# ModelCloud/GPTQModel

Hardware: NVIDIA H100
Metric: W4A16 g128 QuantLinear: decode tok/s + prefill TFLOPS vs HBM/TC roofline (higher is better)
Workload: dtype f16

## Files before the change

gptqmodel_b200/csrc/b2q_gemm.cu:

```cuda
#include <cuda.h>

#include "b2q_common.cuh"
#include "b2q_dequant.cuh"
#include "b2q_gemm.cuh"
#include "b2q_internal.h"
#include "b2q_wgmma.cuh"

namespace b2q {

template <typename T, int BITS, bool ASYM, int STAGES>
__global__ void __launch_bounds__(G_THREADS, 1)
    gemm_kernel(const __grid_constant__ CUtensorMap tmap_x, const __grid_constant__ GemmSets S, int M, int K,
                int gshc) {
  using C = GemmCfg<BITS, STAGES>;
  using E = ET<T>;
  extern __shared__ uint8_t smem_raw[];
  const uint32_t smem_base = (smem_u32(smem_raw) + 1023u) & ~1023u;
  uint8_t* smem = smem_raw + (smem_base - smem_u32(smem_raw));

  const uint32_t sA = smem_base;
  const uint32_t sB = sA + STAGES * C::A_BYTES;
  const uint32_t sP = sB + STAGES * C::B_BYTES;
  const uint32_t sBar = sP + STAGES * C::P_BYTES;
  const uint32_t bar_full = sBar, bar_bready = sBar + 8 * STAGES, bar_empty = sBar + 16 * STAGES;

  int set = 0, tn = blockIdx.x;
  if (S.nsets > 1 && tn >= S.tn_end[0]) {
    set = (S.nsets > 2 && tn >= S.tn_end[1]) ? 2 : 1;
    tn -= S.tn_end[set - 1];
  }
  const int N = S.N[set];
  const uint4* __restrict__ packed = S.packed[set];
  const T* __restrict__ scales = reinterpret_cast<const T*>(S.scales[set]);
  const uint32_t* __restrict__ qzeros = S.qzeros[set];

  const int warp = threadIdx.x >> 5, lane = threadIdx.x & 31;
  const int NT = N >> 5;
  const int n0 = tn * G_BN, m0 = blockIdx.y * G_BM;
  const int nt0 = n0 >> 5;
  const int ntiles = min(4, NT - nt0);
  const int nkb = K / G_BK;

  if (threadIdx.x == 0) {
    prefetch_tmap(&tmap_x);
    for (int s = 0; s < STAGES; ++s) {
      mbar_init(bar_full + 8 * s, 1);
      mbar_init(bar_bready + 8 * s, G_DQ_THREADS);
      mbar_init(bar_empty + 8 * s, 1);
    }
    fence_mbar_init();
  }
  __syncthreads();

  if (warp == 8) {
    if (lane == 0) {
      const int FT = N >> 4, ft0 = n0 >> 4;
      const uint32_t pbytes4 = (uint32_t)min(8, FT - ft0) * 512u;
      const uint32_t pbytes8 = (uint32_t)ntiles * C::SUB * 512u;
      for (int kb = 0; kb < nkb; ++kb) {
        const int s = kb % STAGES;
        const uint32_t ph = (kb / STAGES) & 1;
        mbar_wait(bar_empty + 8 * s, ph ^ 1);
        const int g0 = (2 * kb) >> gshc, g1 = (2 * kb + 1) >> gshc;
        const int nrows = (g1 != g0) ? 2 : 1;
        const uint32_t sbytes = (uint32_t)min(G_BN, N - n0) * 2u, zbytes = ASYM ? sbytes / 4u : 0u;
        mbar_expect_tx(bar_full + 8 * s,
                       C::A_BYTES + (BITS == 4 ? pbytes4 + nrows * (sbytes + zbytes) : 2 * pbytes8));
        tma_load_2d(sA + s * C::A_BYTES, &tmap_x, bar_full + 8 * s, kb * G_BK, m0);
        if (BITS == 4) {
          bulk_load(sP + s * C::P_BYTES, packed + ((size_t)kb * FT + ft0) * 32, pbytes4, bar_full + 8 * s);
          for (int r = 0; r < nrows; ++r) {
            const int gr = r ? g1 : g0;
            bulk_load(sP + s * C::P_BYTES + 4096 + r * 320, scales + (size_t)gr * N + n0, sbytes, bar_full + 8 * s);
            if (ASYM)
              bulk_load(sP + s * C::P_BYTES + 4096 + r * 320 + 256, qzeros + (size_t)gr * (N >> 3) + (n0 >> 3),
                        zbytes, bar_full + 8 * s);
          }
        } else {
#pragma unroll
          for (int j = 0; j < 2; ++j)
            bulk_load(sP + s * C::P_BYTES + j * C::P_CHUNK_BYTES,
                      packed + ((size_t)(kb * 2 + j) * NT + nt0) * C::SUB * 32, pbytes8, bar_full + 8 * s);
        }
      }
    }
  } else if (warp < 4) {
    float acc[2][G_BN / 2];
#pragma unroll
    for (int mb = 0; mb < 2; ++mb)
#pragma unroll
      for (int i = 0; i < G_BN / 2; ++i) acc[mb][i] = 0.f;
    for (int kb = 0; kb < nkb; ++kb) {
      const int s = kb % STAGES;
      const uint32_t ph = (kb / STAGES) & 1;
      mbar_wait(bar_full + 8 * s, ph);
      mbar_wait(bar_bready + 8 * s, ph);
      wgmma_fence();
      const uint64_t bdesc = wgmma_desc_k_sw128(sB + s * C::B_BYTES);
      const uint64_t adesc = wgmma_desc_k_sw128(sA + s * C::A_BYTES);
#pragma unroll
      for (int k = 0; k < G_BK / 16; ++k) {
#pragma unroll
        for (int mb = 0; mb < 2; ++mb)
          Wgmma<E::FMT, G_BN>::mma(acc[mb], adesc + 512 * mb + 2 * k, bdesc + 2 * k, (kb | k) != 0 ? 1u : 0u);
      }
      wgmma_commit();
      wgmma_wait<1>();
      if (kb > 0 && threadIdx.x == 0) mbar_arrive(bar_empty + 8 * ((kb - 1) % STAGES));
    }
    wgmma_wait<0>();
#pragma unroll
    for (int mb = 0; mb < 2; ++mb) wgmma_fence_regs(acc[mb]);

    const T* __restrict__ bias = reinterpret_cast<const T*>(S.bias[set]);
    T* __restrict__ out = reinterpret_cast<T*>(S.out[set]);
#pragma unroll
    for (int mb = 0; mb < 2; ++mb) {
#pragma unroll
      for (int h = 0; h < 2; ++h) {
        const int row = m0 + 64 * mb + 16 * warp + (lane >> 2) + 8 * h;
        if (row >= M) continue;
        T* dst = out + (size_t)row * N;
#pragma unroll
        for (int j = 0; j < G_BN / 8; ++j) {
          const int col = n0 + 8 * j + 2 * (lane & 3);
          if (col >= N) continue;
          float f0 = acc[mb][4 * j + 2 * h], f1 = acc[mb][4 * j + 2 * h + 1];
          if (bias != nullptr) {
            f0 = E::to_f(E::from_f(f0)) + E::to_f(bias[col]);
            f1 = E::to_f(E::from_f(f1)) + E::to_f(bias[col + 1]);
          }
          *reinterpret_cast<uint32_t*>(dst + col) = E::pack2(f0, f1);
        }
      }
    }
  } else {
    const int t = threadIdx.x - G_MMA_THREADS;
    constexpr int PF = 32 / BITS;
    constexpr int ZSYM = 1 << (BITS - 1);
    if (BITS == 4) {
      const int lp = t & 31, g = lp >> 2, tt = lp & 3;
      int f[4];
      f[0] = (t >> 5) * 16 + g;
      f[1] = f[0] + 8;
      f[2] = f[0] + 64;
      f[3] = f[0] + 72;
      for (int kb = 0; kb < nkb; ++kb) {
        const int s = kb % STAGES;
        const uint32_t ph = (kb / STAGES) & 1;
        mbar_wait(bar_full + 8 * s, ph);
        const uint8_t* pst = smem + (sP - smem_base) + s * C::P_BYTES;
        const uint4* pj = reinterpret_cast<const uint4*>(pst);
        const int grow = ((2 * kb + (tt >> 1)) >> gshc) - ((2 * kb) >> gshc);
        const uint8_t* srow = pst + 4096 + grow * 320;
#pragma unroll
        for (int u = 0; u < 2; ++u) {
          const uint4 pv = pj[t + u * 128];
          const uint32_t s_lo = *reinterpret_cast<const uint16_t*>(srow + f[2 * u] * 2);
          const uint32_t s_hi = *reinterpret_cast<const uint16_t*>(srow + f[2 * u + 1] * 2);
          int zl = ZSYM, zh = ZSYM;
          if (ASYM) {
            const uint32_t zwl = *reinterpret_cast<const uint32_t*>(srow + 256 + (f[2 * u] >> 3) * 4);
            const uint32_t zwh = *reinterpret_cast<const uint32_t*>(srow + 256 + (f[2 * u + 1] >> 3) * 4);
            zl = (int)((zwl >> (4 * g)) & 15u);
            zh = (int)((zwh >> (4 * g)) & 15u);
          }
          uint4 lo[2], hi[2];
          Dequant<T, 4>::run(pv, s_lo, zl, s_hi, zh, lo, hi);
          const uint32_t sw = (uint32_t)g;
          const uint32_t rlo = sB + s * C::B_BYTES + f[2 * u] * 128;
          const uint32_t rhi = rlo + 8 * 128;
#pragma unroll
          for (int c = 0; c < 2; ++c) {
            const uint32_t off = (((uint32_t)(2 * tt + c)) ^ sw) << 4;
            asm volatile("st.shared.v4.u32 [%0], {%1,%2,%3,%4};" ::"r"(rlo + off), "r"(lo[c].x), "r"(lo[c].y),
                         "r"(lo[c].z), "r"(lo[c].w)
                         : "memory");
            asm volatile("st.shared.v4.u32 [%0], {%1,%2,%3,%4};" ::"r"(rhi + off), "r"(hi[c].x), "r"(hi[c].y),
                         "r"(hi[c].z), "r"(hi[c].w)
                         : "memory");
          }
        }
        fence_proxy_async_smem();
        mbar_arrive(bar_bready + 8 * s);
      }
    } else {
      const int n = n0 + t;
      const int nsafe = (n < N) ? n : 0;
      const int ntl = t >> 5;
      SZRaw cur[2], nxt[2];
      cur[0] = load_sz<T, BITS, ASYM>(scales, qzeros, 0, nsafe, N);
      cur[1] = load_sz<T, BITS, ASYM>(scales, qzeros, 1 >> gshc, nsafe, N);
      for (int kb = 0; kb < nkb; ++kb) {
        const int s = kb % STAGES;
        const uint32_t ph = (kb / STAGES) & 1;
        if (kb + 1 < nkb) {
          nxt[0] = load_sz<T, BITS, ASYM>(scales, qzeros, (2 * kb + 2) >> gshc, nsafe, N);
          nxt[1] = load_sz<T, BITS, ASYM>(scales, qzeros, (2 * kb + 3) >> gshc, nsafe, N);
        }
        mbar_wait(bar_full + 8 * s, ph);
        const uint32_t brow = sB + s * C::B_BYTES + t * 128;
        const uint32_t sw = (uint32_t)(t & 7);
#pragma unroll
        for (int j = 0; j < 2; ++j) {
          int z = ZSYM;
          if (ASYM) z = (int)((cur[j].zw >> (BITS * (nsafe % PF))) & ((1u << BITS) - 1));
          const uint4* pj = reinterpret_cast<const uint4*>(smem + (sP - smem_base) + s * C::P_BYTES +
                                                           j * C::P_CHUNK_BYTES);
#pragma unroll
          for (int h = 0; h < 2; ++h) {
            const uint4 pv = pj[(ntl * 2 + h) * 32 + lane];
            uint4 o[2];
            Dequant<T, 8>::run(pv, cur[j].s, z, o);
#pragma unroll
            for (int c = 0; c < 2; ++c) {
              const uint32_t addr = brow + (((uint32_t)(j * 4 + h * 2 + c) ^ sw) << 4);
              asm volatile("st.shared.v4.u32 [%0], {%1,%2,%3,%4};" ::"r"(addr), "r"(o[c].x), "r"(o[c].y),
                           "r"(o[c].z), "r"(o[c].w)
                           : "memory");
            }
          }
        }
        fence_proxy_async_smem();
        mbar_arrive(bar_bready + 8 * s);
        cur[0] = nxt[0];
        cur[1] = nxt[1];
      }
    }
  }
}

typedef CUresult (*EncodeTiledFn)(CUtensorMap*, CUtensorMapDataType, cuuint32_t, void*, const cuuint64_t*,
                                  const cuuint64_t*, const cuuint32_t*, const cuuint32_t*, CUtensorMapInterleave,
                                  CUtensorMapSwizzle, CUtensorMapL2promotion, CUtensorMapFloatOOBfill);

static EncodeTiledFn get_encode_fn() {
  static EncodeTiledFn fn = nullptr;
  if (fn == nullptr) {
    void* p = nullptr;
    cudaDriverEntryPointQueryResult qres;
    if (cudaGetDriverEntryPoint("cuTensorMapEncodeTiled", &p, cudaEnableDefault, &qres) == cudaSuccess &&
        qres == cudaDriverEntryPointSuccess)
      fn = reinterpret_cast<EncodeTiledFn>(p);
  }
  return fn;
}

int make_x_tmap_box(CUtensorMap* map, const void* x, int M, int K, int dtype, int box_rows) {
  struct Entry {
    const void* x;
    int M, K, dtype, box;
    CUtensorMap map;
  };
  constexpr int NCACHE = 16;
  static thread_local Entry cache[NCACHE];
  static thread_local int next = 0, filled = 0;
  for (int i = 0; i < filled; ++i) {
    const Entry& c = cache[i];
    if (c.x == x && c.M == M && c.K == K && c.dtype == dtype && c.box == box_rows) {
      *map = c.map;
      return 0;
    }
  }
  EncodeTiledFn enc = get_encode_fn();
  if (enc == nullptr) {
    set_error("b2q_gemm: cuTensorMapEncodeTiled not available from the driver");
    return -1;
  }
  cuuint64_t gdim[2] = {(cuuint64_t)K, (cuuint64_t)M};
  cuuint64_t gstride[1] = {(cuuint64_t)K * 2};
  cuuint32_t box[2] = {(cuuint32_t)G_BK, (cuuint32_t)box_rows};
  cuuint32_t estr[2] = {1, 1};
  CUresult r = enc(map, dtype == 0 ? CU_TENSOR_MAP_DATA_TYPE_FLOAT16 : CU_TENSOR_MAP_DATA_TYPE_BFLOAT16, 2,
                   const_cast<void*>(x), gdim, gstride, box, estr, CU_TENSOR_MAP_INTERLEAVE_NONE,
                   CU_TENSOR_MAP_SWIZZLE_128B, CU_TENSOR_MAP_L2_PROMOTION_L2_256B,
                   CU_TENSOR_MAP_FLOAT_OOB_FILL_NONE);
  if (r != CUDA_SUCCESS) {
    set_error("b2q_gemm: cuTensorMapEncodeTiled failed (%d) for x=%p M=%d K=%d box=%d", (int)r, x, M, K, box_rows);
    return -1;
  }
  Entry& e = cache[next];
  e.x = x;
  e.M = M;
  e.K = K;
  e.dtype = dtype;
  e.box = box_rows;
  e.map = *map;
  next = (next + 1) % NCACHE;
  if (filled < NCACHE) ++filled;
  return 0;
}

int make_x_tmap(CUtensorMap* map, const void* x, int M, int K, int dtype) {
  return make_x_tmap_box(map, x, M, K, dtype, 128);
}

int gemm_gshc(const MmArgs& a) {
  if (a.group_size == 32) return 0;
  if (a.group_size == 64) return 1;
  if (a.group_size == 128) return 2;
  return 31;
}


template <typename T, int BITS, bool ASYM, int STAGES>
static int launch_gemm_t(const MmArgs& a, const void* x, const GemmSets& S) {
  using C = GemmCfg<BITS, STAGES>;
  CUtensorMap tmap;
  if (make_x_tmap(&tmap, x, a.M, a.K, a.dtype) != 0) return -1;
  auto kern = gemm_kernel<T, BITS, ASYM, STAGES>;
  static uint32_t smem_ok = 0;
  if (int e = ensure_dyn_smem(kern, C::SMEM_BYTES, smem_ok, "b2q_gemm")) return e;
  dim3 grid(S.tn_end[S.nsets - 1], (a.M + G_BM - 1) / G_BM, 1);
  kern<<<grid, G_THREADS, C::SMEM_BYTES, a.stream>>>(tmap, S, a.M, a.K, gemm_gshc(a));
  return (int)cudaGetLastError();
}

static int launch_gemm_sets(const MmArgs& a, const void* x, const GemmSets& S) {
  const bool asym = S.qzeros[0] != nullptr;
#define B2Q_GEMM_CASE(T, BITS, ST) \
  (asym ? launch_gemm_t<T, BITS, true, ST>(a, x, S) : launch_gemm_t<T, BITS, false, ST>(a, x, S))
  if (a.dtype == 0) return a.bits == 4 ? B2Q_GEMM_CASE(__half, 4, 4) : B2Q_GEMM_CASE(__half, 8, 4);
  return a.bits == 4 ? B2Q_GEMM_CASE(__nv_bfloat16, 4, 4) : B2Q_GEMM_CASE(__nv_bfloat16, 8, 4);
#undef B2Q_GEMM_CASE
}

int launch_gemm_multi(const MmArgs& a, const void* x, int nsets, const void* const* packed, const void* const* scales,
                      const int32_t* const* qzeros, const void* const* bias, void* const* out, const int* Ns) {
  if (nsets < 1 || nsets > G_MAX_SETS) {
    set_error("b2q_gemm_multi: nsets=%d out of range (1..%d)", nsets, G_MAX_SETS);
    return -1;
  }
  if (a.K % G_BK != 0) {
    set_error("b2q_gemm_multi: K=%d must be a multiple of %d", a.K, G_BK);
    return -1;
  }
  GemmSets S = {};
  S.nsets = nsets;
  int tn = 0;
  for (int i = 0; i < nsets; ++i) {
    if (Ns[i] <= 0 || Ns[i] % 32 != 0 || packed[i] == nullptr || scales[i] == nullptr || out[i] == nullptr ||
        ((qzeros[i] != nullptr) != (qzeros[0] != nullptr))) {
      set_error("b2q_gemm_multi: set %d unsupported (N=%d; all sets share K, group size and symmetry)", i, Ns[i]);
      return -1;
    }
    tn += (Ns[i] + G_BN - 1) / G_BN;
    S.tn_end[i] = tn;
    S.N[i] = Ns[i];
    S.packed[i] = (const uint4*)packed[i];
    S.scales[i] = scales[i];
    S.qzeros[i] = (const uint32_t*)qzeros[i];
    S.bias[i] = bias[i];
    S.out[i] = out[i];
  }
  for (int i = nsets; i < G_MAX_SETS; ++i) S.tn_end[i] = tn;
  return launch_gemm_sets(a, x, S);
}

int launch_gemm(const MmArgs& a) {
  if (a.K % G_BK != 0) {
    set_error("b2q_gemm: K=%d must be a multiple of %d", a.K, G_BK);
    return -1;
  }
  const void* x = a.x;
  if (a.perm != nullptr) {
    const size_t need = (size_t)a.M * a.K * 2;
    if (a.workspace == nullptr || a.workspace_bytes < need) {
      set_error("b2q_gemm: act-order needs a %zu-byte workspace (got %zu)", need, a.workspace_bytes);
      return -1;
    }
    int e = launch_permute_cols(a.x, a.perm, a.workspace, a.M, a.K, a.stream);
    if (e != 0) return e;
    x = a.workspace;
  }
  if (a.M <= 128 && env().midm && midm_supported(a)) return launch_midm(a, x);
  const void* packed = a.packed;
  const void* scales = a.scales;
  const int32_t* qzeros = (const int32_t*)a.qzeros;
  const void* bias = a.bias;
  void* out = a.out;
  return launch_gemm_multi(a, x, 1, &packed, &scales, &qzeros, &bias, &out, &a.N);
}

}
```

gptqmodel_b200/csrc/b2q_gemm.cuh:

```cuda
#pragma once
#include "b2q_common.cuh"

namespace b2q {

constexpr int G_BM = 128;
constexpr int G_BN = 128;
constexpr int G_BK = 64;
constexpr int G_MMA_THREADS = 128;
constexpr int G_DQ_THREADS = 128;
constexpr int G_THREADS = G_MMA_THREADS + G_DQ_THREADS + 32;

template <int BITS, int STAGES>
struct GemmCfg {
  static constexpr int SUB = BITS / 4;
  static constexpr int A_BYTES = G_BM * G_BK * 2;
  static constexpr int B_BYTES = G_BN * G_BK * 2;
  static constexpr int P_CHUNK_BYTES = 4 * SUB * 512;
  static constexpr int P_BYTES = 2 * P_CHUNK_BYTES + (BITS == 4 ? 1024 : 0);
  static constexpr int STAGE_BYTES = A_BYTES + B_BYTES + P_BYTES;
  static constexpr int BAR_BYTES = 256;
  static constexpr int SMEM_BYTES = STAGES * STAGE_BYTES + BAR_BYTES + 1024;
  static_assert(SMEM_BYTES <= 227 * 1024, "dynamic shared memory of one CTA");
};

constexpr int G_MAX_SETS = 3;
struct GemmSets {
  int nsets;
  int tn_end[G_MAX_SETS];
  int N[G_MAX_SETS];
  const uint4* packed[G_MAX_SETS];
  const void* scales[G_MAX_SETS];
  const uint32_t* qzeros[G_MAX_SETS];
  const void* bias[G_MAX_SETS];
  void* out[G_MAX_SETS];
};

}
```

Baseline: 619.9.

## Make W4A16 GEMM persistent with L2-banded tile order and smem-staged epilogue

```diff
diff --git a/gptqmodel_b200/csrc/b2q_gemm.cu b/gptqmodel_b200/csrc/b2q_gemm.cu
--- a/gptqmodel_b200/csrc/b2q_gemm.cu
+++ b/gptqmodel_b200/csrc/b2q_gemm.cu
@@ -1,4 +1,6 @@
 #include <cuda.h>
+
+#include <algorithm>
 
 #include "b2q_common.cuh"
 #include "b2q_dequant.cuh"
@@ -7,6 +9,31 @@
 #include "b2q_wgmma.cuh"
 
 namespace b2q {
+
+struct GemmTile {
+  int set;
+  int n0;
+  int m0;
+  int N;
+};
+
+__device__ __forceinline__ GemmTile gemm_tile(const GemmSets& S, int idx, int ncols, int mblocks) {
+  const int per_band = S.band * ncols;
+  const int b = idx / per_band;
+  const int r = idx - b * per_band;
+  const int rows = min(S.band, mblocks - b * S.band);
+  int tn = r / rows;
+  GemmTile t;
+  t.m0 = (b * S.band + (r - tn * rows)) * G_BM;
+  t.set = 0;
+  if (S.nsets > 1 && tn >= S.tn_end[0]) {
+    t.set = (S.nsets > 2 && tn >= S.tn_end[1]) ? 2 : 1;
+    tn -= S.tn_end[t.set - 1];
+  }
+  t.n0 = tn * G_BN;
+  t.N = S.N[t.set];
+  return t;
+}
 
 template <typename T, int BITS, bool ASYM, int STAGES>
 __global__ void __launch_bounds__(G_THREADS, 1)
@@ -21,24 +48,14 @@
   const uint32_t sA = smem_base;
   const uint32_t sB = sA + STAGES * C::A_BYTES;
   const uint32_t sP = sB + STAGES * C::B_BYTES;
-  const uint32_t sBar = sP + STAGES * C::P_BYTES;
+  const uint32_t sO = sP + STAGES * C::P_BYTES;
+  const uint32_t sBar = sO + C::OUT_BYTES;
   const uint32_t bar_full = sBar, bar_bready = sBar + 8 * STAGES, bar_empty = sBar + 16 * STAGES;
 
-  int set = 0, tn = blockIdx.x;
-  if (S.nsets > 1 && tn >= S.tn_end[0]) {
-    set = (S.nsets > 2 && tn >= S.tn_end[1]) ? 2 : 1;
-    tn -= S.tn_end[set - 1];
-  }
-  const int N = S.N[set];
-  const uint4* __restrict__ packed = S.packed[set];
-  const T* __restrict__ scales = reinterpret_cast<const T*>(S.scales[set]);
-  const uint32_t* __restrict__ qzeros = S.qzeros[set];
-
   const int warp = threadIdx.x >> 5, lane = threadIdx.x & 31;
-  const int NT = N >> 5;
-  const int n0 = tn * G_BN, m0 = blockIdx.y * G_BM;
-  const int nt0 = n0 >> 5;
-  const int ntiles = min(4, NT - nt0);
+  const int ncols = S.tn_end[S.nsets - 1];
+  const int mblocks = (M + G_BM - 1) / G_BM;
+  const int ntile = ncols * mblocks;
   const int nkb = K / G_BK;
 
   if (threadIdx.x == 0) {
@@ -54,33 +71,42 @@
 
   if (warp == 8) {
     if (lane == 0) {
-      const int FT = N >> 4, ft0 = n0 >> 4;
-      const uint32_t pbytes4 = (uint32_t)min(8, FT - ft0) * 512u;
-      const uint32_t pbytes8 = (uint32_t)ntiles * C::SUB * 512u;
-      for (int kb = 0; kb < nkb; ++kb) {
-        const int s = kb % STAGES;
-        const uint32_t ph = (kb / STAGES) & 1;
-        mbar_wait(bar_empty + 8 * s, ph ^ 1);
-        const int g0 = (2 * kb) >> gshc, g1 = (2 * kb + 1) >> gshc;
-        const int nrows = (g1 != g0) ? 2 : 1;
+      uint32_t it = 0;
+      for (int idx = blockIdx.x; idx < ntile; idx += gridDim.x) {
+        const GemmTile tl = gemm_tile(S, idx, ncols, mblocks);
+        const int N = tl.N, n0 = tl.n0, m0 = tl.m0;
+        const uint4* __restrict__ packed = S.packed[tl.set];
+        const T* __restrict__ scales = reinterpret_cast<const T*>(S.scales[tl.set]);
+        const uint32_t* __restrict__ qzeros = S.qzeros[tl.set];
+        const int NT = N >> 5, nt0 = n0 >> 5;
+        const int FT = N >> 4, ft0 = n0 >> 4;
+        const uint32_t pbytes4 = (uint32_t)min(8, FT - ft0) * 512u;
+        const uint32_t pbytes8 = (uint32_t)min(4, NT - nt0) * C::SUB * 512u;
         const uint32_t sbytes = (uint32_t)min(G_BN, N - n0) * 2u, zbytes = ASYM ? sbytes / 4u : 0u;
-        mbar_expect_tx(bar_full + 8 * s,
-                       C::A_BYTES + (BITS == 4 ? pbytes4 + nrows * (sbytes + zbytes) : 2 * pbytes8));
-        tma_load_2d(sA + s * C::A_BYTES, &tmap_x, bar_full + 8 * s, kb * G_BK, m0);
-        if (BITS == 4) {
-          bulk_load(sP + s * C::P_BYTES, packed + ((size_t)kb * FT + ft0) * 32, pbytes4, bar_full + 8 * s);
-          for (int r = 0; r < nrows; ++r) {
-            const int gr = r ? g1 : g0;
-            bulk_load(sP + s * C::P_BYTES + 4096 + r * 320, scales + (size_t)gr * N + n0, sbytes, bar_full + 8 * s);
-            if (ASYM)
-              bulk_load(sP + s * C::P_BYTES + 4096 + r * 320 + 256, qzeros + (size_t)gr * (N >> 3) + (n0 >> 3),
-                        zbytes, bar_full + 8 * s);
-          }
-        } else {
-#pragma unroll
-          for (int j = 0; j < 2; ++j)
-            bulk_load(sP + s * C::P_BYTES + j * C::P_CHUNK_BYTES,
-                      packed + ((size_t)(kb * 2 + j) * NT + nt0) * C::SUB * 32, pbytes8, bar_full + 8 * s);
+        for (int kb = 0; kb < nkb; ++kb, ++it) {
+          const int s = it % STAGES;
+          const uint32_t ph = (it / STAGES) & 1;
+          mbar_wait(bar_empty + 8 * s, ph ^ 1);
+          const int g0 = (2 * kb) >> gshc, g1 = (2 * kb + 1) >> gshc;
+          const int nrows = (g1 != g0) ? 2 : 1;
+          mbar_expect_tx(bar_full + 8 * s,
+                         C::A_BYTES + (BITS == 4 ? pbytes4 + nrows * (sbytes + zbytes) : 2 * pbytes8));
+          tma_load_2d(sA + s * C::A_BYTES, &tmap_x, bar_full + 8 * s, kb * G_BK, m0);
+          if (BITS == 4) {
+            bulk_load(sP + s * C::P_BYTES, packed + ((size_t)kb * FT + ft0) * 32, pbytes4, bar_full + 8 * s);
+            for (int r = 0; r < nrows; ++r) {
+              const int gr = r ? g1 : g0;
+              bulk_load(sP + s * C::P_BYTES + 4096 + r * 320, scales + (size_t)gr * N + n0, sbytes, bar_full + 8 * s);
+              if (ASYM)
+                bulk_load(sP + s * C::P_BYTES + 4096 + r * 320 + 256, qzeros + (size_t)gr * (N >> 3) + (n0 >> 3),
+                          zbytes, bar_full + 8 * s);
+            }
+          } else {
+#pragma unroll
+            for (int j = 0; j < 2; ++j)
+              bulk_load(sP + s * C::P_BYTES + j * C::P_CHUNK_BYTES,
+                        packed + ((size_t)(kb * 2 + j) * NT + nt0) * C::SUB * 32, pbytes8, bar_full + 8 * s);
+          }
         }
       }
     }
@@ -90,47 +116,79 @@
     for (int mb = 0; mb < 2; ++mb)
 #pragma unroll
       for (int i = 0; i < G_BN / 2; ++i) acc[mb][i] = 0.f;
-    for (int kb = 0; kb < nkb; ++kb) {
-      const int s = kb % STAGES;
-      const uint32_t ph = (kb / STAGES) & 1;
-      mbar_wait(bar_full + 8 * s, ph);
-      mbar_wait(bar_bready + 8 * s, ph);
-      wgmma_fence();
-      const uint64_t bdesc = wgmma_desc_k_sw128(sB + s * C::B_BYTES);
-      const uint64_t adesc = wgmma_desc_k_sw128(sA + s * C::A_BYTES);
-#pragma unroll
-      for (int k = 0; k < G_BK / 16; ++k) {
-#pragma unroll
-        for (int mb = 0; mb < 2; ++mb)
-          Wgmma<E::FMT, G_BN>::mma(acc[mb], adesc + 512 * mb + 2 * k, bdesc + 2 * k, (kb | k) != 0 ? 1u : 0u);
-      }
-      wgmma_commit();
-      wgmma_wait<1>();
-      if (kb > 0 && threadIdx.x == 0) mbar_arrive(bar_empty + 8 * ((kb - 1) % STAGES));
-    }
-    wgmma_wait<0>();
-#pragma unroll
-    for (int mb = 0; mb < 2; ++mb) wgmma_fence_regs(acc[mb]);
-
-    const T* __restrict__ bias = reinterpret_cast<const T*>(S.bias[set]);
-    T* __restrict__ out = reinterpret_cast<T*>(S.out[set]);
-#pragma unroll
-    for (int mb = 0; mb < 2; ++mb) {
-#pragma unroll
-      for (int h = 0; h < 2; ++h) {
-        const int row = m0 + 64 * mb + 16 * warp + (lane >> 2) + 8 * h;
-        if (row >= M) continue;
-        T* dst = out + (size_t)row * N;
-#pragma unroll
-        for (int j = 0; j < G_BN / 8; ++j) {
-          const int col = n0 + 8 * j + 2 * (lane & 3);
-          if (col >= N) continue;
-          float f0 = acc[mb][4 * j + 2 * h], f1 = acc[mb][4 * j + 2 * h + 1];
-          if (bias != nullptr) {
-            f0 = E::to_f(E::from_f(f0)) + E::to_f(bias[col]);
-            f1 = E::to_f(E::from_f(f1)) + E::to_f(bias[col + 1]);
-          }
-          *reinterpret_cast<uint32_t*>(dst + col) = E::pack2(f0, f1);
+    uint32_t it = 0;
+    for (int idx = blockIdx.x; idx < ntile; idx += gridDim.x) {
+      for (int kb = 0; kb < nkb; ++kb, ++it) {
+        const int s = it % STAGES;
+        const uint32_t ph = (it / STAGES) & 1;
+        mbar_wait(bar_full + 8 * s, ph);
+        mbar_wait(bar_bready + 8 * s, ph);
+        wgmma_fence();
+        const uint64_t bdesc = wgmma_desc_k_sw128(sB + s * C::B_BYTES);
+        const uint64_t adesc = wgmma_desc_k_sw128(sA + s * C::A_BYTES);
+#pragma unroll
+        for (int k = 0; k < G_BK / 16; ++k) {
+#pragma unroll
+          for (int mb = 0; mb < 2; ++mb)
+            Wgmma<E::FMT, G_BN>::mma(acc[mb], adesc + 512 * mb + 2 * k, bdesc + 2 * k, (kb | k) != 0 ? 1u : 0u);
+        }
+        wgmma_commit();
+        wgmma_wait<1>();
+        if (kb > 0 && threadIdx.x == 0) mbar_arrive(bar_empty + 8 * ((it - 1) % STAGES));
+      }
+      wgmma_wait<0>();
+#pragma unroll
+      for (int mb = 0; mb < 2; ++mb) wgmma_fence_regs(acc[mb]);
+      if (threadIdx.x == 0) mbar_arrive(bar_empty + 8 * ((it - 1) % STAGES));
+
+      GemmTile tl = gemm_tile(S, idx, ncols, mblocks);
+      const T* __restrict__ bias = reinterpret_cast<const T*>(S.bias[tl.set]);
+      if (bias != nullptr) bias += tl.n0 + 2 * (lane & 3);
+      const int ncol = tl.N - tl.n0 - 2 * (lane & 3);
+      asm volatile("bar.sync 1, %0;" ::"n"(G_MMA_THREADS) : "memory");
+#pragma unroll
+      for (int mb = 0; mb < 2; ++mb) {
+#pragma unroll
+        for (int h = 0; h < 2; ++h) {
+          const int r = 64 * mb + 16 * warp + (lane >> 2) + 8 * h;
+          const uint32_t srow = sO + r * G_OUT_ROW + 4 * (lane & 3);
+#pragma unroll
+          for (int j = 0; j < G_BN / 8; ++j) {
+            float f0 = acc[mb][4 * j + 2 * h], f1 = acc[mb][4 * j + 2 * h + 1];
+            if (bias != nullptr && 8 * j < ncol) {
+              f0 = E::to_f(E::from_f(f0)) + E::to_f(bias[8 * j]);
+              f1 = E::to_f(E::from_f(f1)) + E::to_f(bias[8 * j + 1]);
+            }
+            asm volatile("st.shared.u32 [%0], %1;" ::"r"(srow + 16 * j), "r"(E::pack2(f0, f1)) : "memory");
+          }
+        }
+      }
+      asm volatile("bar.sync 1, %0;" ::"n"(G_MMA_THREADS) : "memory");
+      tl = gemm_tile(S, idx, ncols, mblocks);
+      const int N = tl.N, n0 = tl.n0, m0 = tl.m0;
+      T* __restrict__ out = reinterpret_cast<T*>(S.out[tl.set]);
+      const bool vec = (reinterpret_cast<uintptr_t>(out) & 15u) == 0;
+      const int c = threadIdx.x & 15;
+#pragma unroll 4
+      for (int i = 0; i < G_BM / 8; ++i) {
+        const int r = 8 * i + (threadIdx.x >> 4);
+        const int row = m0 + r, col = n0 + 8 * c;
+        if (row < M && col < N) {
+          uint4 v;
+          asm volatile("ld.shared.v4.u32 {%0,%1,%2,%3}, [%4];"
+                       : "=r"(v.x), "=r"(v.y), "=r"(v.z), "=r"(v.w)
+                       : "r"(sO + r * G_OUT_ROW + 16 * c)
+                       : "memory");
+          T* dst = out + (size_t)row * N + col;
+          if (vec) {
+            *reinterpret_cast<uint4*>(dst) = v;
+          } else {
+            uint32_t* d32 = reinterpret_cast<uint32_t*>(dst);
+            d32[0] = v.x;
+            d32[1] = v.y;
+            d32[2] = v.z;
+            d32[3] = v.w;
+          }
         }
       }
     }
@@ -138,6 +196,7 @@
     const int t = threadIdx.x - G_MMA_THREADS;
     constexpr int PF = 32 / BITS;
     constexpr int ZSYM = 1 << (BITS - 1);
+    uint32_t it = 0;
     if (BITS == 4) {
       const int lp = t & 31, g = lp >> 2, tt = lp & 3;
       int f[4];
@@ -145,86 +204,94 @@
       f[1] = f[0] + 8;
       f[2] = f[0] + 64;
       f[3] = f[0] + 72;
-      for (int kb = 0; kb < nkb; ++kb) {
-        const int s = kb % STAGES;
-        const uint32_t ph = (kb / STAGES) & 1;
-        mbar_wait(bar_full + 8 * s, ph);
-        const uint8_t* pst = smem + (sP - smem_base) + s * C::P_BYTES;
-        const uint4* pj = reinterpret_cast<const uint4*>(pst);
-        const int grow = ((2 * kb + (tt >> 1)) >> gshc) - ((2 * kb) >> gshc);
-        const uint8_t* srow = pst + 4096 + grow * 320;
-#pragma unroll
-        for (int u = 0; u < 2; ++u) {
-          const uint4 pv = pj[t + u * 128];
-          const uint32_t s_lo = *reinterpret_cast<const uint16_t*>(srow + f[2 * u] * 2);
-          const uint32_t s_hi = *reinterpret_cast<const uint16_t*>(srow + f[2 * u + 1] * 2);
-          int zl = ZSYM, zh = ZSYM;
-          if (ASYM) {
-            const uint32_t zwl = *reinterpret_cast<const uint32_t*>(srow + 256 + (f[2 * u] >> 3) * 4);
-            const uint32_t zwh = *reinterpret_cast<const uint32_t*>(srow + 256 + (f[2 * u + 1] >> 3) * 4);
-            zl = (int)((zwl >> (4 * g)) & 15u);
-            zh = (int)((zwh >> (4 * g)) & 15u);
-          }
-          uint4 lo[2], hi[2];
-          Dequant<T, 4>::run(pv, s_lo, zl, s_hi, zh, lo, hi);
-          const uint32_t sw = (uint32_t)g;
-          const uint32_t rlo = sB + s * C::B_BYTES + f[2 * u] * 128;
-          const uint32_t rhi = rlo + 8 * 128;
-#pragma unroll
-          for (int c = 0; c < 2; ++c) {
-            const uint32_t off = (((uint32_t)(2 * tt + c)) ^ sw) << 4;
-            asm volatile("st.shared.v4.u32 [%0], {%1,%2,%3,%4};" ::"r"(rlo + off), "r"(lo[c].x), "r"(lo[c].y),
-                         "r"(lo[c].z), "r"(lo[c].w)
-                         : "memory");
-            asm volatile("st.shared.v4.u32 [%0], {%1,%2,%3,%4};" ::"r"(rhi + off), "r"(hi[c].x), "r"(hi[c].y),
-                         "r"(hi[c].z), "r"(hi[c].w)
-                         : "memory");
-          }
-        }
-        fence_proxy_async_smem();
-        mbar_arrive(bar_bready + 8 * s);
-      }
-    } else {
-      const int n = n0 + t;
-      const int nsafe = (n < N) ? n : 0;
-      const int ntl = t >> 5;
-      SZRaw cur[2], nxt[2];
-      cur[0] = load_sz<T, BITS, ASYM>(scales, qzeros, 0, nsafe, N);
-      cur[1] = load_sz<T, BITS, ASYM>(scales, qzeros, 1 >> gshc, nsafe, N);
-      for (int kb = 0; kb < nkb; ++kb) {
-        const int s = kb % STAGES;
-        const uint32_t ph = (kb / STAGES) & 1;
-        if (kb + 1 < nkb) {
-          nxt[0] = load_sz<T, BITS, ASYM>(scales, qzeros, (2 * kb + 2) >> gshc, nsafe, N);
-          nxt[1] = load_sz<T, BITS, ASYM>(scales, qzeros, (2 * kb + 3) >> gshc, nsafe, N);
-        }
-        mbar_wait(bar_full + 8 * s, ph);
-        const uint32_t brow = sB + s * C::B_BYTES + t * 128;
-        const uint32_t sw = (uint32_t)(t & 7);
-#pragma unroll
-        for (int j = 0; j < 2; ++j) {
-          int z = ZSYM;
-          if (ASYM) z = (int)((cur[j].zw >> (BITS * (nsafe % PF))) & ((1u << BITS) - 1));
-          const uint4* pj = reinterpret_cast<const uint4*>(smem + (sP - smem_base) + s * C::P_BYTES +
-                                                           j * C::P_CHUNK_BYTES);
-#pragma unroll
-          for (int h = 0; h < 2; ++h) {
-            const uint4 pv = pj[(ntl * 2 + h) * 32 + lane];
-            uint4 o[2];
-            Dequant<T, 8>::run(pv, cur[j].s, z, o);
+      for (int idx = blockIdx.x; idx < ntile; idx += gridDim.x) {
+        for (int kb = 0; kb < nkb; ++kb, ++it) {
+          const int s = it % STAGES;
+          const uint32_t ph = (it / STAGES) & 1;
+          mbar_wait(bar_full + 8 * s, ph);
+          const uint8_t* pst = smem + (sP - smem_base) + s * C::P_BYTES;
+          const uint4* pj = reinterpret_cast<const uint4*>(pst);
+          const int grow = ((2 * kb + (tt >> 1)) >> gshc) - ((2 * kb) >> gshc);
+          const uint8_t* srow = pst + 4096 + grow * 320;
+#pragma unroll
+          for (int u = 0; u < 2; ++u) {
+            const uint4 pv = pj[t + u * 128];
+            const uint32_t s_lo = *reinterpret_cast<const uint16_t*>(srow + f[2 * u] * 2);
+            const uint32_t s_hi = *reinterpret_cast<const uint16_t*>(srow + f[2 * u + 1] * 2);
+            int zl = ZSYM, zh = ZSYM;
+            if (ASYM) {
+              const uint32_t zwl = *reinterpret_cast<const uint32_t*>(srow + 256 + (f[2 * u] >> 3) * 4);
+              const uint32_t zwh = *reinterpret_cast<const uint32_t*>(srow + 256 + (f[2 * u + 1] >> 3) * 4);
+              zl = (int)((zwl >> (4 * g)) & 15u);
+              zh = (int)((zwh >> (4 * g)) & 15u);
+            }
+            uint4 lo[2], hi[2];
+            Dequant<T, 4>::run(pv, s_lo, zl, s_hi, zh, lo, hi);
+            const uint32_t sw = (uint32_t)g;
+            const uint32_t rlo = sB + s * C::B_BYTES + f[2 * u] * 128;
+            const uint32_t rhi = rlo + 8 * 128;
 #pragma unroll
             for (int c = 0; c < 2; ++c) {
-              const uint32_t addr = brow + (((uint32_t)(j * 4 + h * 2 + c) ^ sw) << 4);
-              asm volatile("st.shared.v4.u32 [%0], {%1,%2,%3,%4};" ::"r"(addr), "r"(o[c].x), "r"(o[c].y),
-                           "r"(o[c].z), "r"(o[c].w)
+              const uint32_t off = (((uint32_t)(2 * tt + c)) ^ sw) << 4;
+              asm volatile("st.shared.v4.u32 [%0], {%1,%2,%3,%4};" ::"r"(rlo + off), "r"(lo[c].x), "r"(lo[c].y),
+                           "r"(lo[c].z), "r"(lo[c].w)
+                           : "memory");
+              asm volatile("st.shared.v4.u32 [%0], {%1,%2,%3,%4};" ::"r"(rhi + off), "r"(hi[c].x), "r"(hi[c].y),
+                           "r"(hi[c].z), "r"(hi[c].w)
                            : "memory");
             }
           }
-        }
-        fence_proxy_async_smem();
-        mbar_arrive(bar_bready + 8 * s);
-        cur[0] = nxt[0];
-        cur[1] = nxt[1];
+          fence_proxy_async_smem();
+          mbar_arrive(bar_bready + 8 * s);
+        }
+      }
+    } else {
+      const int ntl = t >> 5;
+      for (int idx = blockIdx.x; idx < ntile; idx += gridDim.x) {
+        const GemmTile tl = gemm_tile(S, idx, ncols, mblocks);
+        const int N = tl.N;
+        const T* __restrict__ scales = reinterpret_cast<const T*>(S.scales[tl.set]);
+        const uint32_t* __restrict__ qzeros = S.qzeros[tl.set];
+        const int n = tl.n0 + t;
+        const int nsafe = (n < N) ? n : 0;
+        SZRaw cur[2], nxt[2];
+        cur[0] = load_sz<T, BITS, ASYM>(scales, qzeros, 0, nsafe, N);
+        cur[1] = load_sz<T, BITS, ASYM>(scales, qzeros, 1 >> gshc, nsafe, N);
+        for (int kb = 0; kb < nkb; ++kb, ++it) {
+          const int s = it % STAGES;
+          const uint32_t ph = (it / STAGES) & 1;
+          if (kb + 1 < nkb) {
+            nxt[0] = load_sz<T, BITS, ASYM>(scales, qzeros, (2 * kb + 2) >> gshc, nsafe, N);
+            nxt[1] = load_sz<T, BITS, ASYM>(scales, qzeros, (2 * kb + 3) >> gshc, nsafe, N);
+          }
+          mbar_wait(bar_full + 8 * s, ph);
+          const uint32_t brow = sB + s * C::B_BYTES + t * 128;
+          const uint32_t sw = (uint32_t)(t & 7);
+#pragma unroll
+          for (int j = 0; j < 2; ++j) {
+            int z = ZSYM;
+            if (ASYM) z = (int)((cur[j].zw >> (BITS * (nsafe % PF))) & ((1u << BITS) - 1));
+            const uint4* pj = reinterpret_cast<const uint4*>(smem + (sP - smem_base) + s * C::P_BYTES +
+                                                             j * C::P_CHUNK_BYTES);
+#pragma unroll
+            for (int h = 0; h < 2; ++h) {
+              const uint4 pv = pj[(ntl * 2 + h) * 32 + lane];
+              uint4 o[2];
+              Dequant<T, 8>::run(pv, cur[j].s, z, o);
+#pragma unroll
+              for (int c = 0; c < 2; ++c) {
+                const uint32_t addr = brow + (((uint32_t)(j * 4 + h * 2 + c) ^ sw) << 4);
+                asm volatile("st.shared.v4.u32 [%0], {%1,%2,%3,%4};" ::"r"(addr), "r"(o[c].x), "r"(o[c].y),
+                             "r"(o[c].z), "r"(o[c].w)
+                             : "memory");
+              }
+            }
+          }
+          fence_proxy_async_smem();
+          mbar_arrive(bar_bready + 8 * s);
+          cur[0] = nxt[0];
+          cur[1] = nxt[1];
+        }
       }
     }
   }
@@ -303,6 +370,32 @@
 }
 
 
+static long long l2_bytes() {
+  static long long cache[32] = {};
+  int dev = 0;
+  if (cudaGetDevice(&dev) != cudaSuccess || dev < 0 || dev >= 32) {
+    (void)cudaGetLastError();
+    return 50ll << 20;
+  }
+  if (cache[dev] == 0) {
+    int n = 0;
+    if (cudaDeviceGetAttribute(&n, cudaDevAttrL2CacheSize, dev) != cudaSuccess || n <= 0) {
+      (void)cudaGetLastError();
+      n = 50 << 20;
+    }
+    cache[dev] = n;
+  }
+  return cache[dev];
+}
+
+static int gemm_band(int M, int K) {
+  const int mblocks = (M + G_BM - 1) / G_BM;
+  const long long blk = (long long)G_BM * K * 2;
+  const long long maxb = std::max(1ll, (l2_bytes() / 2) / blk);
+  const int nb = (int)((mblocks + maxb - 1) / maxb);
+  return (mblocks + nb - 1) / nb;
+}
+
 template <typename T, int BITS, bool ASYM, int STAGES>
 static int launch_gemm_t(const MmArgs& a, const void* x, const GemmSets& S) {
   using C = GemmCfg<BITS, STAGES>;
@@ -311,7 +404,8 @@
   auto kern = gemm_kernel<T, BITS, ASYM, STAGES>;
   static uint32_t smem_ok = 0;
   if (int e = ensure_dyn_smem(kern, C::SMEM_BYTES, smem_ok, "b2q_gemm")) return e;
-  dim3 grid(S.tn_end[S.nsets - 1], (a.M + G_BM - 1) / G_BM, 1);
+  const int tiles = S.tn_end[S.nsets - 1] * ((a.M + G_BM - 1) / G_BM);
+  const int grid = std::min(tiles, num_sms());
   kern<<<grid, G_THREADS, C::SMEM_BYTES, a.stream>>>(tmap, S, a.M, a.K, gemm_gshc(a));
   return (int)cudaGetLastError();
 }
@@ -320,8 +414,8 @@
   const bool asym = S.qzeros[0] != nullptr;
 #define B2Q_GEMM_CASE(T, BITS, ST) \
   (asym ? launch_gemm_t<T, BITS, true, ST>(a, x, S) : launch_gemm_t<T, BITS, false, ST>(a, x, S))
-  if (a.dtype == 0) return a.bits == 4 ? B2Q_GEMM_CASE(__half, 4, 4) : B2Q_GEMM_CASE(__half, 8, 4);
-  return a.bits == 4 ? B2Q_GEMM_CASE(__nv_bfloat16, 4, 4) : B2Q_GEMM_CASE(__nv_bfloat16, 8, 4);
+  if (a.dtype == 0) return a.bits == 4 ? B2Q_GEMM_CASE(__half, 4, 5) : B2Q_GEMM_CASE(__half, 8, 4);
+  return a.bits == 4 ? B2Q_GEMM_CASE(__nv_bfloat16, 4, 5) : B2Q_GEMM_CASE(__nv_bfloat16, 8, 4);
 #undef B2Q_GEMM_CASE
 }
 
@@ -354,6 +448,7 @@
     S.out[i] = out[i];
   }
   for (int i = nsets; i < G_MAX_SETS; ++i) S.tn_end[i] = tn;
+  S.band = gemm_band(a.M, a.K);
   return launch_gemm_sets(a, x, S);
 }
 
diff --git a/gptqmodel_b200/csrc/b2q_gemm.cuh b/gptqmodel_b200/csrc/b2q_gemm.cuh
--- a/gptqmodel_b200/csrc/b2q_gemm.cuh
+++ b/gptqmodel_b200/csrc/b2q_gemm.cuh
@@ -9,6 +9,7 @@
 constexpr int G_MMA_THREADS = 128;
 constexpr int G_DQ_THREADS = 128;
 constexpr int G_THREADS = G_MMA_THREADS + G_DQ_THREADS + 32;
+constexpr int G_OUT_ROW = G_BN * 2 + 16;
 
 template <int BITS, int STAGES>
 struct GemmCfg {
@@ -18,8 +19,9 @@
   static constexpr int P_CHUNK_BYTES = 4 * SUB * 512;
   static constexpr int P_BYTES = 2 * P_CHUNK_BYTES + (BITS == 4 ? 1024 : 0);
   static constexpr int STAGE_BYTES = A_BYTES + B_BYTES + P_BYTES;
+  static constexpr int OUT_BYTES = G_BM * G_OUT_ROW;
   static constexpr int BAR_BYTES = 256;
-  static constexpr int SMEM_BYTES = STAGES * STAGE_BYTES + BAR_BYTES + 1024;
+  static constexpr int SMEM_BYTES = STAGES * STAGE_BYTES + OUT_BYTES + BAR_BYTES + 1024;
   static_assert(SMEM_BYTES <= 227 * 1024, "dynamic shared memory of one CTA");
 };
 
@@ -33,6 +35,7 @@
   const uint32_t* qzeros[G_MAX_SETS];
   const void* bias[G_MAX_SETS];
   void* out[G_MAX_SETS];
+  int band;
 };
 
 }
```

After: 620.0, median of 6. No clear change (+0.0%).
